# prs-eth/PCAccumulation

Hardware: AMD Instinct MI355X
Metric: LiDAR-frames/sec (5-frame seq, 160k pts) fwd+bwd (higher is better)
Workload: dtype mixed

## Files before the change

### include/pcacc.h

```cpp
#ifndef PCACC_H_
#define PCACC_H_

#include <stddef.h>
#include <stdint.h>

#ifdef __cplusplus
extern "C" {
#endif

#define PCACC_OK 0
#define PCACC_E_ARG (-1)
#define PCACC_E_WORKSPACE (-2)
#define PCACC_E_LAUNCH (-3)

#define PCACC_F32 0
#define PCACC_BF16 1

const char *pcacc_target(void);

int pcacc_cat2_rows(const void *a, int32_t a_row_bytes, const void *b, int32_t b_row_bytes, int64_t rows, void *out, void *stream);

int pcacc_reload_switches(void);

int pcacc_voxelize_workspace_bytes(int64_t n, int nx, int ny, int nz, int nt, size_t *bytes );
// ... 330 lines not shown

int pcacc_frames_max(const void *x, int dtype, int64_t n_seq, int32_t frames, int64_t plane, void *out, uint8_t *arg, void *stream);
int pcacc_frames_max_backward(const void *grad_out, const uint8_t *arg, int dtype, int64_t n_seq, int32_t frames, int64_t plane,
                              void *grad_x, void *stream);

int pcacc_bn_rows_workspace_bytes(int64_t rows, int32_t c, size_t *bytes );
int pcacc_bn_rows_forward(const void *x, int dtype, int64_t rows, int32_t c, const float *gamma, const float *beta, float eps,
                          float momentum, float *running_mean, float *running_var, void *y, float *save_mean,
                          float *save_invstd, void *workspace, size_t workspace_bytes, void *stream);
int pcacc_bn_rows_backward(const void *grad_y, const void *x, int dtype, int64_t rows, int32_t c, const float *gamma,
                           const float *save_mean, const float *save_invstd, void *grad_x, float *grad_gamma, float *grad_beta,
                           void *workspace, size_t workspace_bytes, void *stream);

int pcacc_bn_relu_rows_forward(const void *x, int dtype, int64_t rows, int32_t c, const float *gamma, const float *beta, float eps,
                               float momentum, float *running_mean, float *running_var, void *y, float *save_mean, float *save_invstd,
                               void *workspace, size_t workspace_bytes, void *stream);
int pcacc_bn_relu_rows_backward(const void *grad_y, const void *x, int dtype, int64_t rows, int32_t c, const float *gamma, const float *beta,
                                const float *save_mean, const float *save_invstd, void *grad_x, float *grad_gamma, float *grad_beta,
                                void *workspace, size_t workspace_bytes, void *stream);
int pcacc_bn_rows_forward_dual(const float *x, int64_t rows, int32_t c, const float *gamma, const float *beta, float eps, float momentum,
                               float *running_mean, float *running_var, int32_t relu, float *y, uint16_t *y16, float *y_amax, float *save_mean,
                               float *save_invstd, void *workspace, size_t workspace_bytes, void *stream);

int pcacc_bn_rows_backward_m(const void *grad_y, const void *x, int dtype, int64_t rows, int32_t c, const float *gamma, const float *beta,
                             int32_t relu, const float *save_mean, const float *save_invstd, void *grad_x, float *grad_x_amax, float *grad_gamma,
                             float *grad_beta, void *workspace, size_t workspace_bytes, void *stream);

int pcacc_pfn_block_forward(const uint16_t *xa, const uint16_t *pooled, const int32_t *p2v, const float *w0, const float *b0,
                            const float *ws, const float *w1, const float *b1, uint16_t *out, uint16_t *relu_h, int64_t rows, void *stream);
int pcacc_pfn_block_backward_workspace_bytes(int64_t rows, size_t *bytes );
int pcacc_pfn_block_backward(const uint16_t *xa, const uint16_t *pooled, const int32_t *p2v, const uint16_t *relu_h,
                             const uint16_t *grad_out, const float *w0, const float *ws, const float *w1, uint16_t *grad_xa,
                             uint16_t *grad_xb, float *grad_params, int64_t rows, void *workspace, size_t workspace_bytes, void *stream);

int pcacc_pfn_block_split_forward(const float *xa, const float *xa_amax, const float *pooled, const float *pooled_amax, const int32_t *p2v,
                                  const float *w0, const float *b0, const float *ws, const float *w1, const float *b1, float *out,
                                  float *relu_h, uint64_t *xmask, uint32_t *hmask, float *out_amax, float *hr_amax, int64_t rows,
                                  void *stream);
int pcacc_pfn_block_split_forward_dual(const float *xa, const float *xa_amax, const float *pooled, const float *pooled_amax, const int32_t *p2v,
                                       const float *w0, const float *b0, const float *ws, const float *w1, const float *b1, float *out,
                                       uint16_t *out16, uint16_t *hr16, float *out_amax, int64_t rows, void *stream);
int pcacc_pfn_block_split_dgrad(const float *grad_out, const float *grad_out_amax, const uint64_t *xmask, const uint32_t *hmask,
                                const float *w0, const float *ws, const float *w1, float *grad_xa, float *grad_xb, float *grad_h,
                                float *gx_amax, float *dh_amax, int64_t rows, void *stream);

int pcacc_maxpool2x2_bf16(const uint16_t *x, int64_t n_img, int32_t h, int32_t w, int32_t c, uint16_t *out, void *stream);
int pcacc_pool_skip_relu_backward_bf16(const uint16_t *y, const uint16_t *grad_pooled, const uint16_t *grad_skip, int64_t n_img, int32_t h,
                                       int32_t w, int32_t c, uint16_t *grad_y, void *stream);
int pcacc_maxpool2x2_f32(const float *x, int64_t n_img, int32_t h, int32_t w, int32_t c, float *out, void *stream);
int pcacc_pool_skip_relu_backward_f32(const float *y, const float *grad_pooled, const float *grad_skip, int64_t n_img, int32_t h, int32_t w,
                                      int32_t c, float *grad_y, float *out_amax, void *stream);
int pcacc_pool_skip_relu_backward_strided_bf16(const uint16_t *y, const uint16_t *grad_pooled, const uint16_t *grad_skip, int64_t skip_pitch,
                                               int64_t n_img, int32_t h, int32_t w, int32_t c, uint16_t *grad_y, void *stream);
int pcacc_pool_skip_relu_backward_strided_f32(const float *y, const float *grad_pooled, const float *grad_skip, int64_t skip_pitch,
                                              int64_t n_img, int32_t h, int32_t w, int32_t c, float *grad_y, float *out_amax, void *stream);
int pcacc_pool_skip_relu_backward_strided_y32(const float *y, const uint16_t *grad_pooled, const uint16_t *grad_skip, int64_t skip_pitch,
                                              int64_t n_img, int32_t h, int32_t w, int32_t c, uint16_t *grad_y, void *stream);

int pcacc_inv4x4(const float *m, int64_t n, float *out, void *stream);

int pcacc_rows_wgrad_few_supported(int32_t k, int32_t n);
int pcacc_rows_wgrad_few_workspace_bytes(int64_t rows, int32_t k, int32_t n, size_t *bytes );
int pcacc_rows_wgrad_few(const void *dy, const void *dy_mask, const void *x, int32_t x_relu, int64_t rows, int32_t k, int32_t n,
                         float *dw_aug, int32_t dtypes, void *workspace, size_t workspace_bytes, void *stream);

int pcacc_tube_rows(const float *xyz, const int32_t *slot, const float *slot_centre, int64_t n, int32_t n_frames, float *rows, void *stream);
int pcacc_tube_code(const float *geo, const float *motion, const float *frame, int64_t n_inst, int32_t n_frames, int32_t c, float *code,
                    void *stream);
int pcacc_tube_code_backward(const float *grad_code, int64_t n_inst, int32_t n_frames, int32_t c, float *grad_geo, float *grad_motion,
                             float *grad_frame, void *stream);
int pcacc_tube_pose_forward(const float *pose_vec, const float *remaining, const float *total_in, const float *slot_centre,
                            const float *weights, int32_t n_slots, int32_t n_frames, float *pose_c, float *gt_c, float *step,
                            float *remaining_out, float *total_out, double *loss_rt, float *wsum, void *stream);
int pcacc_tube_gap_forward(const float *rows, const int32_t *slot, const float *pose_c, const float *gt_c, int64_t n, float *pp, void *stream);
int pcacc_tube_finish(const float *slot_sums, int32_t stride, const float *count, const float *weights, const float *wsum, int32_t n_slots,
                      float *l12, void *stream);
int pcacc_tube_gap_backward(const float *rows, const int32_t *slot, const float *pose_c, const float *gt_c, const float *weights,
                            const float *count, const float *wsum, const float *grad_l1, const float *grad_l2, int64_t n,
                            float *grad_rows16, void *stream);
int pcacc_tube_pose_backward(const float *pose_vec, const float *remaining, const float *slot_centre, const float *weights, const float *wsum,
                             const float *grad_pose, int32_t stride, const double *grad_rot, const double *grad_trans, int32_t n_slots,
                             int32_t n_frames, float *grad_vec, void *stream);

int pcacc_upload_words(const uint32_t *host_words, int64_t n, uint32_t *dst, void *stream);

#ifdef __cplusplus
}
#endif
#endif
```

### pcaccumulation_amd/native.py

```python
import ctypes
import os
import re

import torch

_HERE = os.path.dirname(os.path.abspath(__file__))
LIB_PATH = os.environ.get('PCACC_LIB') or os.path.join(_HERE, 'csrc', 'libpcacc_hip.so')

F32, BF16 = 0, 1
_ERR = {-1: 'PCACC_E_ARG', -2: 'PCACC_E_WORKSPACE', -3: 'PCACC_E_LAUNCH'}

_lib = None


class NativeError(RuntimeError):
    pass


_CTYPES = {'int': ctypes.c_int, 'int32_t': ctypes.c_int, 'int64_t': ctypes.c_int64, 'uint64_t': ctypes.c_uint64, 'size_t': ctypes.c_size_t,
           'float': ctypes.c_float, 'double': ctypes.c_double}


def _prototypes():
    text = re.sub(r'/\*.*?\*/', '', open(os.path.join(_HERE, os.pardir, 'include', 'pcacc.h')).read(), flags=re.S)
# ... 1379 lines not shown
    _check(lib().pcacc_bn_rows_backward(_dev(grad_y, None, 'grad_y'), _dev(x, None, 'x'), _dtype_code(x), rows, int(c),
                                        _opt(gamma, torch.float32, 'gamma'), _dev(save_mean, torch.float32), _dev(save_invstd, torch.float32),
                                        _dev(gx), _dev(gg), _dev(gb), _dev(ws), ws.numel(), _stream()), 'bn_rows_backward')
    return gx, gg, gb


def tube_rows(xyz, slot, slot_centre, n_frames):
    n = xyz.shape[0]
    rows = torch.empty((n, 4), dtype=torch.float32, device=xyz.device)
    _check(lib().pcacc_tube_rows(_dev(xyz, torch.float32, 'xyz'), _dev(slot, torch.int32, 'slot'), _dev(slot_centre, torch.float32, 'slot_centre'),
                                 n, int(n_frames), _dev(rows), _stream()), 'tube_rows')
    return rows


def tube_code(geo, motion, frame, n_frames):
    n_inst, c = geo.shape
    code = torch.empty((n_inst * n_frames, 4 * c), dtype=torch.float32, device=geo.device)
    _check(lib().pcacc_tube_code(_dev(geo, torch.float32, 'geo'), _dev(motion, torch.float32, 'motion'), _dev(frame, torch.float32, 'frame'),
                                 n_inst, int(n_frames), int(c), _dev(code), _stream()), 'tube_code')
    return code


def tube_code_backward(grad_code, n_inst, n_frames, c):
    dev = grad_code.device
    g_geo = torch.empty((n_inst, c), dtype=torch.float32, device=dev)
    g_motion = torch.empty((n_inst, c), dtype=torch.float32, device=dev)
    g_frame = torch.empty((n_inst * n_frames, c), dtype=torch.float32, device=dev)
    _check(lib().pcacc_tube_code_backward(_dev(grad_code, torch.float32, 'grad_code'), n_inst, int(n_frames), int(c), _dev(g_geo),
                                          _dev(g_motion), _dev(g_frame), _stream()), 'tube_code_backward')
    return g_geo, g_motion, g_frame


def tube_pose_forward(pose_vec, remaining, total, slot_centre, weights, n_frames):
    s = pose_vec.shape[0]
    dev = pose_vec.device
    f = lambda *shape: torch.empty(shape, dtype=torch.float32, device=dev)
    pose_c, gt_c, step, rem_out, total_out, wsum = f(s, 12), f(s, 12), f(s, 4, 4), f(s, 4, 4), f(s, 4, 4), f(1)
    loss_rt = torch.empty((2,), dtype=torch.float64, device=dev)
    _check(lib().pcacc_tube_pose_forward(_dev(pose_vec, torch.float32, 'pose_vec'), _dev(remaining, torch.float32, 'remaining'),
                                         _opt(total, torch.float32, 'total'), _dev(slot_centre, torch.float32, 'slot_centre'),
                                         _dev(weights, torch.float32, 'weights'), int(s), int(n_frames), _dev(pose_c), _dev(gt_c), _dev(step),
                                         _dev(rem_out), _dev(total_out), _dev(loss_rt), _dev(wsum), _stream()), 'tube_pose_forward')
    return pose_c, gt_c, step, rem_out, total_out, loss_rt, wsum


def tube_gap_forward(rows, slot, pose_c, gt_c):
    n = rows.shape[0]
    pp = torch.empty((n, 4), dtype=torch.float32, device=rows.device)
    _check(lib().pcacc_tube_gap_forward(_dev(rows, torch.float32, 'rows'), _dev(slot, torch.int32, 'slot'), _dev(pose_c, torch.float32, 'pose_c'),
                                        _dev(gt_c, torch.float32, 'gt_c'), n, _dev(pp), _stream()), 'tube_gap_forward')
    return pp


def tube_finish(slot_sums, count, weights, wsum):
    l12 = torch.empty((2,), dtype=torch.float32, device=slot_sums.device)
    _check(lib().pcacc_tube_finish(_dev(slot_sums, torch.float32, 'slot_sums'), int(slot_sums.shape[1]), _dev(count, torch.float32, 'count'),
                                   _dev(weights, torch.float32, 'weights'), _dev(wsum, torch.float32, 'wsum'), int(slot_sums.shape[0]),
                                   _dev(l12), _stream()), 'tube_finish')
    return l12


def tube_gap_backward(rows, slot, pose_c, gt_c, weights, count, wsum, grad_l1, grad_l2):
    n = rows.shape[0]
    g16 = torch.empty((n, 16), dtype=torch.float32, device=rows.device)
    _check(lib().pcacc_tube_gap_backward(_dev(rows, torch.float32, 'rows'), _dev(slot, torch.int32, 'slot'), _dev(pose_c, torch.float32, 'pose_c'),
                                         _dev(gt_c, torch.float32, 'gt_c'), _dev(weights, torch.float32, 'weights'),
                                         _dev(count, torch.float32, 'count'), _dev(wsum, torch.float32, 'wsum'),
                                         _opt(grad_l1, torch.float32, 'grad_l1'), _opt(grad_l2, torch.float32, 'grad_l2'), n, _dev(g16),
                                         _stream()), 'tube_gap_backward')
    return g16


def tube_pose_backward(pose_vec, remaining, slot_centre, weights, wsum, grad_pose, grad_rot, grad_trans, n_frames):
    s = pose_vec.shape[0]
    g_vec = torch.empty((s, 7), dtype=torch.float32, device=pose_vec.device)
    _check(lib().pcacc_tube_pose_backward(_dev(pose_vec, torch.float32, 'pose_vec'), _dev(remaining, torch.float32, 'remaining'),
                                          _dev(slot_centre, torch.float32, 'slot_centre'), _dev(weights, torch.float32, 'weights'),
                                          _dev(wsum, torch.float32, 'wsum'), _dev(grad_pose, torch.float32, 'grad_pose'), int(grad_pose.shape[1]),
                                          _opt(grad_rot, torch.float64, 'grad_rot'), _opt(grad_trans, torch.float64, 'grad_trans'), int(s),
                                          int(n_frames), _dev(g_vec), _stream()), 'tube_pose_backward')
    return g_vec


def maxpool2x2(x_rows):
    n, h, w, c = x_rows.shape
    out = torch.empty((n, h // 2, w // 2, c), dtype=x_rows.dtype, device=x_rows.device)
    if x_rows.dtype == torch.float32:
        _check(lib().pcacc_maxpool2x2_f32(_dev(x_rows, torch.float32, 'x'), n, int(h), int(w), int(c), _dev(out), _stream()), 'maxpool2x2')
    else:
        _check(lib().pcacc_maxpool2x2_bf16(_dev(x_rows, torch.bfloat16, 'x'), n, int(h), int(w), int(c), _dev(out), _stream()), 'maxpool2x2')
    return out


def _pixel_pitch(g, shape):
    n, h, w, c = shape
    if tuple(g.shape) != tuple(shape) or g.stride(3) != 1:
        return None
    p = g.stride(2)
    if p < c or g.stride(1) != w * p or g.stride(0) != h * w * p or g.data_ptr() % 16:
        return None
    return p


def pool_skip_relu_backward(y_rows, grad_pooled, grad_skip, want_amax=False):
    n, h, w, c = y_rows.shape
    if y_rows.dtype == torch.float32 and any(g is not None and g.dtype == torch.bfloat16 for g in (grad_pooled, grad_skip)):
        out = torch.empty(y_rows.shape, dtype=torch.bfloat16, device=y_rows.device)
        pitch, gs_ptr = c, None
        if grad_skip is not None:
            pitch = _pixel_pitch(grad_skip, y_rows.shape)
            if pitch is None or pitch % 8:
                grad_skip, pitch = grad_skip.contiguous(), c
            gs_ptr = ctypes.c_void_p(grad_skip.data_ptr())
        _check(lib().pcacc_pool_skip_relu_backward_strided_y32(_dev(y_rows, torch.float32, 'y'), _opt(grad_pooled, torch.bfloat16, 'grad_pooled'), gs_ptr,
                                                               pitch, n, int(h), int(w), int(c), _dev(out), _stream()), 'pool_skip_relu_backward')
        return out
    out = torch.empty_like(y_rows)
    f32 = y_rows.dtype == torch.float32
    dt = torch.float32 if f32 else torch.bfloat16
    pitch, gs_ptr = c, None
    if grad_skip is not None:
        if grad_skip.dtype != dt or not grad_skip.is_cuda:
            raise NativeError('pool_skip_relu_backward: grad_skip must be a %s GPU tensor' % dt)
        pitch = _pixel_pitch(grad_skip, y_rows.shape)
        if pitch is None or pitch % (4 if f32 else 8):
            grad_skip, pitch = grad_skip.contiguous(), c
        gs_ptr = ctypes.c_void_p(grad_skip.data_ptr())
    if f32:
        amax = _zero256(y_rows.device) if want_amax else None
        _check(lib().pcacc_pool_skip_relu_backward_strided_f32(_dev(y_rows, torch.float32, 'y'), _opt(grad_pooled, torch.float32, 'grad_pooled'), gs_ptr,
                                                               pitch, n, int(h), int(w), int(c), _dev(out),
                                                               _dev(amax) if want_amax else None, _stream()), 'pool_skip_relu_backward')
        return (out, amax) if want_amax else out
    _check(lib().pcacc_pool_skip_relu_backward_strided_bf16(_dev(y_rows, torch.bfloat16, 'y'), _opt(grad_pooled, torch.bfloat16, 'grad_pooled'), gs_ptr,
                                                            pitch, n, int(h), int(w), int(c), _dev(out), _stream()), 'pool_skip_relu_backward')
    return out


PFN_BLOCK_SLICES = {'w1': (0, 1024, (32, 32)), 'b1': (1024, 1056, (32,)), 'ws': (1056, 3104, (32, 64)), 'w0': (3104, 5152, (32, 64)),
                    'b0': (5152, 5184, (32,))}


def pfn_block_forward(xa, pooled, p2v, w0, b0, ws, w1, b1):
    rows = xa.shape[0]
    out = torch.empty((rows, 32), dtype=torch.bfloat16, device=xa.device)
    hr = torch.empty((rows, 32), dtype=torch.bfloat16, device=xa.device)
    _check(lib().pcacc_pfn_block_forward(_dev(xa, torch.bfloat16, 'xa'), _opt(pooled, torch.bfloat16, 'pooled'), _opt(p2v, torch.int32, 'p2v'),
                                         _dev(w0, torch.float32, 'w0'), _opt(b0, torch.float32, 'b0'), _dev(ws, torch.float32, 'ws'),
                                         _dev(w1, torch.float32, 'w1'), _opt(b1, torch.float32, 'b1'), _dev(out), _dev(hr), rows, _stream()), 'pfn_block_forward')
    return out, hr


def pfn_block_backward(xa, pooled, p2v, hr, grad_out, w0, ws, w1):
    rows = xa.shape[0]
    dev = xa.device
    two = pooled is not None
    gxa = torch.empty((rows, 32 if two else 64), dtype=torch.bfloat16, device=dev)
    gxb = torch.empty((rows, 32), dtype=torch.bfloat16, device=dev) if two else None
    gp = torch.empty((5184,), dtype=torch.float32, device=dev)
    ws_buf = _workspace(lib().pcacc_pfn_block_backward_workspace_bytes, dev, rows)
    _check(lib().pcacc_pfn_block_backward(_dev(xa, torch.bfloat16, 'xa'), _opt(pooled, torch.bfloat16, 'pooled'), _opt(p2v, torch.int32, 'p2v'),
                                          _dev(hr, torch.bfloat16, 'relu_h'), _dev(grad_out, torch.bfloat16, 'grad_out'),
                                          _dev(w0, torch.float32, 'w0'), _dev(ws, torch.float32, 'ws'), _dev(w1, torch.float32, 'w1'),
                                          _dev(gxa), _opt(gxb, torch.bfloat16, 'grad_xb'), _dev(gp), rows, _dev(ws_buf),
                                          ws_buf.numel(), _stream()), 'pfn_block_backward')
    return gxa, gxb, gp
# ... 134 lines not shown
```

### pcaccumulation_amd/ops.py

```python
import weakref

import os

import torch

from . import native


class PillarIndex(object):

    def __init__(self, coordinates, point_to_voxel_map, batch_size, input_shape, cell_order=False):
        nx, ny, nz, nt = (int(v) for v in input_shape[:4])
        self.nx, self.ny, self.nt, self.batch_size = nx, ny, nt, int(batch_size)
        self.m = int(coordinates.shape[0])
        self.n_cells = self.batch_size * nt * ny * nx
        self.cells_per_frame = ny * nx
        coords = coordinates.contiguous()
        if coords.dtype not in (torch.float64, torch.int32):
            coords = coords.to(torch.float64)
        self.cell, self.cell2pillar = native.cell_index(coords, nx, ny, nt, self.batch_size)
        self.coordinates, self.perm, self._frames = coordinates, None, None
        p2v = point_to_voxel_map
        if p2v is not None:
            p2v = (p2v[:, 0] if p2v.dim() == 2 else p2v).to(torch.int32)
# ... 912 lines not shown
    def forward(ctx, points, idx, tsfm):
        tsfm = tsfm.detach().clone()
        ctx.save_for_backward(points, idx, tsfm)
        return native.rigid_transform(points, idx, tsfm.reshape(-1, 16))

    @staticmethod
    def backward(ctx, g):
        points, idx, tsfm = ctx.saved_tensors
        g = g.contiguous()
        gp = gt = None
        if ctx.needs_input_grad[0]:
            rt = torch.zeros_like(tsfm)
            rt[:, :3, :3] = tsfm[:, :3, :3].transpose(1, 2)
            gp = native.rigid_transform(g, idx, rt.reshape(-1, 16).contiguous())
        if ctx.needs_input_grad[2]:
            hom = torch.cat([points, torch.ones_like(points[:, :1])], dim=1)
            outer = (g[:, :, None] * hom[:, None, :]).reshape(-1, 12)
            rows = scatter(outer, idx, dim=0, dim_size=tsfm.shape[0], reduce='sum')
            gt = torch.zeros_like(tsfm)
            gt[:, :3, :] = rows.view(-1, 3, 4)
        return gp, None, gt


def transform_by_index(points, idx, tsfm):
    out = _TransformByIndex.apply(points.contiguous().float(), idx.to(torch.int32).contiguous(), tsfm.contiguous().float())
    return out if points.dtype == torch.float32 else out.to(points.dtype)


def _plan_sum(x, plan):
    if plan.small(x.shape[1]):
        return native.scatter_sum_small(x, plan.p2v, plan.m)
    return native.segment_sum(x, plan.seg_offsets, plan.order, plan.m)


def tube_rows(xyz, plan, slot_centre, n_frames):
    return native.tube_rows(xyz.detach().contiguous().float(), plan.p2v, slot_centre.detach().contiguous().float(), n_frames)


class _TubeCode(torch.autograd.Function):
    @staticmethod
    def forward(ctx, geo, motion, frame, n_frames):
        ctx.dims = (geo.shape[0], n_frames, geo.shape[1])
        return native.tube_code(geo.contiguous(), motion.contiguous(), frame.contiguous(), n_frames)

    @staticmethod
    def backward(ctx, grad):
        g_geo, g_motion, g_frame = native.tube_code_backward(grad.contiguous(), *ctx.dims)
        return g_geo, g_motion, g_frame, None


def tube_code(geo, motion, frame, n_frames):
    return _TubeCode.apply(geo.float(), motion.float(), frame.float(), int(n_frames))


class _TubePose(torch.autograd.Function):

    @staticmethod
    def forward(ctx, pose_vec, rows, plan, remaining, total, slot_centre, weights, n_frames):
        pose_vec = pose_vec.contiguous().float()
        remaining = remaining.detach().contiguous().float().view(-1, 4, 4)
        total = total.detach().contiguous().float().view(-1, 4, 4) if total is not None else None
        pose_c, gt_c, step, rem_out, total_out, loss_rt, wsum = native.tube_pose_forward(pose_vec, remaining, total, slot_centre, weights, n_frames)
        count = plan.count()
        l12 = native.tube_finish(_plan_sum(native.tube_gap_forward(rows, plan.p2v, pose_c, gt_c), plan), count, weights, wsum)
        ctx.save_for_backward(pose_vec, rows, remaining, slot_centre, weights, pose_c, gt_c, count, wsum)
        ctx.plan, ctx.n_frames = plan, n_frames
        ctx.mark_non_differentiable(step, rem_out, total_out)
        return l12[0], l12[1], loss_rt[0], loss_rt[1], step, rem_out, total_out

    @staticmethod
    def backward(ctx, g_l1, g_l2, g_rot, g_trans, *unused):
        pose_vec, rows, remaining, slot_centre, weights, pose_c, gt_c, count, wsum = ctx.saved_tensors
        plan = ctx.plan
        c = lambda g, dt: g.contiguous().to(dt) if g is not None else None
        g16 = native.tube_gap_backward(rows, plan.p2v, pose_c, gt_c, weights, count, wsum, c(g_l1, torch.float32), c(g_l2, torch.float32))
        g_vec = native.tube_pose_backward(pose_vec, remaining, slot_centre, weights, wsum, _plan_sum(g16, plan), c(g_rot, torch.float64),
                                          c(g_trans, torch.float64), ctx.n_frames)
        return g_vec, None, None, None, None, None, None, None


def tube_pose(pose_vec, rows, plan, remaining, total, slot_centre, weights, n_frames):
    return _TubePose.apply(pose_vec, rows, plan, remaining, total, slot_centre.detach().contiguous().float(), weights.detach().contiguous().float(),
                           int(n_frames))


_PREPARED = {}
_WEIGHT_EPOCH = 0


def weights_may_have_changed():
    global _WEIGHT_EPOCH
    _WEIGHT_EPOCH += 1


_ALL_OPTIMIZERS_WATCHED = False


def watch_all_optimizers():
    global _ALL_OPTIMIZERS_WATCHED
    if not _ALL_OPTIMIZERS_WATCHED:
        from torch.optim.optimizer import register_optimizer_step_post_hook
        register_optimizer_step_post_hook(lambda *a, **k: weights_may_have_changed())
        _ALL_OPTIMIZERS_WATCHED = True


def _weight_key(weight):
    return (weight._version, weight.data_ptr(), _WEIGHT_EPOCH)


def _weight_ref(cache, key, weight):
    return weakref.ref(weight, lambda _r, c=cache, k=key: c.pop(k, None))


_BATCH_ON = os.environ.get('PCACC_BATCH_PREPARE', '1') != '0'
_BATCH_SEEN = {}
_BATCH_STATE = {}


def _batch_note(weight, kind):
    k = (id(weight), kind)
    if _BATCH_ON and k not in _BATCH_SEEN and weight.is_cuda and weight.dtype == torch.float32:
        _BATCH_SEEN[k] = weakref.ref(weight, lambda _r, k=k: _BATCH_SEEN.pop(k, None))


def _batch_build(dev, live):
    import numpy as np
    jobs = np.zeros((len(live), 16), dtype=np.int64)
    forms, b0 = [], 0
    for row, (ref, w, kind) in zip(jobs, live):
        st = w.stride()
        if kind == 1:
            a, b, kt = w.shape[0], w.shape[1], 1
            fwd = (torch.empty((2, 4 * b, a), dtype=torch.float16, device=dev), torch.empty((4 * b,), dtype=torch.float32, device=dev))
            bwd = (torch.empty((2, a, 4 * b), dtype=torch.float16, device=dev), torch.empty((a,), dtype=torch.float32, device=dev))
            strides, blocks = (st[0], st[1], 0, st[2], st[3]), 4 * b + a
        elif kind == 3:
            a, b, kt = w.shape[0], w.shape[1], 1
            fwd = torch.empty((4 * b, a), dtype=torch.bfloat16, device=dev)
            bwd = torch.empty((a, 4 * b), dtype=torch.bfloat16, device=dev)
            strides, blocks = (st[0], st[1], 0, st[2], st[3]), min(512, max(1, (8 * a * b + 2047) // 2048))
        else:
            a, b, kt = w.shape[0], w.shape[1], (3 if w.dim() == 5 else 1)
            strides = tuple(st) if kt == 3 else (st[0], st[1], 0, st[2], st[3])
            if kind == 0:
                fwd = (torch.empty((2, kt * 9, a, b), dtype=torch.float16, device=dev), torch.empty((a,), dtype=torch.float32, device=dev))
                bwd = (torch.empty((2, kt * 9, b, a), dtype=torch.float16, device=dev), torch.empty((b,), dtype=torch.float32, device=dev))
                blocks = a + b
            else:
                fwd = torch.empty((kt * 9, a, b), dtype=torch.bfloat16, device=dev)
                bwd = torch.empty((kt * 9, b, a), dtype=torch.bfloat16, device=dev)
                blocks = min(512, max(1, (2 * kt * 9 * a * b + 2047) // 2048))
        ptrs = (fwd[0].data_ptr(), fwd[1].data_ptr(), bwd[0].data_ptr(), bwd[1].data_ptr()) if kind < 2 else (fwd.data_ptr(), 0, bwd.data_ptr(), 0)
        row[:] = (w.data_ptr(),) + ptrs + strides + (a, b, kt, kind, b0, blocks)
        b0 += blocks
        forms.append((ref, kind, fwd, bwd))
    return {'jobs': torch.from_numpy(jobs).to(dev), 'n': len(live), 'blocks': b0, 'forms': forms}


def _batch_refresh(dev):
    state = _BATCH_STATE.get(dev.index)
    if state is not None and state['epoch'] == _WEIGHT_EPOCH:
        return False
    live = []
    for (_, kind), ref in list(_BATCH_SEEN.items()):
        w = ref()
        if w is not None and w.is_cuda and w.device == dev and w.dtype == torch.float32:
# ... 899 lines not shown
```

### pcaccumulation_amd/tpointnet.py

```python
import torch
import torch.nn as nn
import torch.nn.functional as F

from .chamfer_distance import ChamferDistance
from . import ops
from .ops import scatter, ScatterPlan, linear_rows, transform_by_index, point_dtype, tube_rows, tube_code, tube_pose

_EPS = 1e-20


_CONST = {}


def _const(name, device, build):
    key = (name, str(device))
    if key not in _CONST:
        _CONST[key] = build().to(device)
    return _CONST[key]


def _quat_products_to_pose():
    x, y, z, w = 0, 1, 2, 3
    rot = {(0, 0): [(w, w, 1), (x, x, 1), (y, y, -1), (z, z, -1)], (0, 1): [(x, y, 2), (w, z, -2)], (0, 2): [(w, y, 2), (x, z, 2)],
           (1, 0): [(w, z, 2), (x, y, 2)], (1, 1): [(w, w, 1), (x, x, -1), (y, y, 1), (z, z, -1)], (1, 2): [(y, z, 2), (w, x, -2)],
# ... 124 lines not shown
    layers = []
    for i in range(len(dims) - 1):
        layers.append(nn.Linear(dims[i], dims[i + 1], bias=True))
        if i < len(dims) - 2:
            layers.append(nn.ReLU())
    return nn.Sequential(*layers)


def _embed(seq, x):
    mods = list(seq)
    i = 0
    pd = point_dtype() if x.is_cuda else x.dtype
    if pd != x.dtype and mods[0].in_features >= 32:
        x = x.to(pd)
    head = False
    n_lin = sum(isinstance(m, nn.Linear) for m in mods)
    if ops.mixed_mode() and x.is_cuda and x.dtype == torch.float32 and x.shape[0] >= ops.MIN_ROWS_FUSED_LINEAR and n_lin > 1:
        if mods[0].in_features >= 32:
            x = ops.enter_mixed(x.contiguous())
        else:
            head = True
    k = 0
    while i < len(mods):
        relu = i + 1 < len(mods) and isinstance(mods[i + 1], nn.ReLU)
        k += 1
        if k == n_lin:
            x = ops.exit_mixed(x)
        x = linear_rows(x, mods[i], post_relu=relu, out_dtype=pd, mixed=head and i == 0)
        i += 2 if relu else 1
    return x


class TPointNet(BaseModel):

    def __init__(self, config):
        BaseModel.__init__(self, config)
        self.geo_embed = _mlp([32, 32, 64, 128])
        self.motion_embed = _mlp([64, 64, 128, 128])
        self.pos_embed = _mlp([4, 32, 64, 128])
        self.regressor = nn.Sequential(nn.Linear(512, 256), nn.BatchNorm1d(256), nn.ReLU(),
                                       nn.Linear(256, 128), nn.BatchNorm1d(128), nn.ReLU(), nn.Linear(128, 7))
        self.min_points_per_frame = config['tpointnet']['min_points']

    def _frame_weights(self, slot, per_slot, moving, n_inst, n_slots, device):
        ones = torch.ones(slot.size(0), device=device)
        population = scatter(ones, slot, dim=0, dim_size=n_slots, reduce='sum', plan=per_slot)
        enough = (population > self.min_points_per_frame).float()
        slot_label = scatter(moving, slot, dim=0, dim_size=n_slots, reduce='max', plan=per_slot)
        label_w = torch.ones_like(slot_label)
        label_w[slot_label == 0] = 0.2
        ramp = (torch.arange(self.n_frames, device=device) + 1).repeat(n_inst) / self.n_frames
        return enough * label_w * ramp

    def shared_terms(self, input_dict):
        feats_motion, feats_geo = input_dict['mos_feats'], input_dict['frame_feats']
        t_idx, inst = input_dict['time_indice'], input_dict['inst_labels']
        n_inst, T = input_dict['inst_motion_gt'].size(0), input_dict['inst_motion_gt'].size(1)
        n_slots = n_inst * T
        slot = (inst * T + t_idx).long()
        per_slot = ScatterPlan(slot, n_slots)
        per_inst = ScatterPlan(inst, n_inst)
        weights = self._frame_weights(slot, per_slot, input_dict['mos_labels'], n_inst, n_slots, feats_motion.device)
        e_motion = scatter(_embed(self.motion_embed, feats_motion), inst, dim=0, dim_size=n_inst, reduce='max', plan=per_inst)
        e_geo = scatter(_embed(self.geo_embed, feats_geo), inst, dim=0, dim_size=n_inst, reduce='max', plan=per_inst)
        return {'slot': slot, 'per_slot': per_slot, 'per_inst': per_inst, 'weights': weights,
                'e_motion': e_motion.float(), 'e_geo': e_geo.float()}

    def _frame_embedding(self, xyz, slot, per_slot, n_slots, T):
        slot_centre = scatter(xyz, slot, dim=0, dim_size=n_slots, reduce='mean', plan=per_slot)
        rows = tube_rows(xyz, per_slot, slot_centre, T)
        e_frame = scatter(_embed(self.pos_embed, rows), slot, dim=0, dim_size=n_slots, reduce='max', plan=per_slot)
        return e_frame.float(), slot_centre, rows

    def forward(self, input_dict, shared=None):
        xyz = input_dict['points']
        gt_motion = input_dict['inst_motion_gt']
        n_inst, T = gt_motion.size(0), gt_motion.size(1)
        n_slots = n_inst * T
        if shared is None:
            shared = self.shared_terms(input_dict)
        slot, per_slot, weights = shared['slot'], shared['per_slot'], shared['weights']
        e_frame, slot_centre, rows = self._frame_embedding(xyz, slot, per_slot, n_slots, T)

        pose_vec = self.regressor(tube_code(shared['e_geo'], shared['e_motion'], e_frame, T))

        l1_loss, l2_loss, rot_loss, trans_loss, step, remaining, total = tube_pose(
            pose_vec, rows, per_slot, gt_motion, input_dict.get('total'), slot_centre, weights, T)
        shape = (n_inst, T, 4, 4)
        return {'l1_loss': l1_loss, 'l2_loss': l2_loss, 'rot_loss': rot_loss, 'trans_loss': trans_loss,
                'inst_est_motion': step.view(shape), 'remaining': remaining.view(shape), 'total': total.view(shape)}
```

Baseline: 668.0.

## Fuse tube regressor MLP with BatchNorm and ReLU into custom HIP kernels

```diff
diff --git a/include/pcacc.h b/include/pcacc.h
--- a/include/pcacc.h
+++ b/include/pcacc.h
@@ -436,6 +436,18 @@
                              const float *grad_pose, int32_t stride, const double *grad_rot, const double *grad_trans, int32_t n_slots,
                              int32_t n_frames, float *grad_vec, void *stream);
 
+int pcacc_tube_regressor_forward(const float *x, int64_t m, const float *w1, const float *b1, const float *gamma1, const float *beta1, float eps1,
+                                 float momentum1, float *running_mean1, float *running_var1, int64_t *num_batches_tracked1, const float *w2,
+                                 const float *b2, const float *gamma2, const float *beta2, float eps2, float momentum2, float *running_mean2,
+                                 float *running_var2, int64_t *num_batches_tracked2, const float *w3, const float *b3, float *z1, float *y1,
+                                 float *mean1, float *invstd1, float *z2, float *y2, float *mean2, float *invstd2, float *pose, void *stream);
+int pcacc_tube_regressor_backward(const float *grad_pose, const float *x, int64_t m, const float *w1, const float *gamma1, const float *w2,
+                                  const float *gamma2, const float *w3, const float *z1, const float *y1, const float *mean1,
+                                  const float *invstd1, const float *z2, const float *y2, const float *mean2, const float *invstd2, float *gz1,
+                                  float *gz2, float *grad_x, float *grad_w1, float *grad_b1, float *grad_gamma1, float *grad_beta1,
+                                  float *grad_w2, float *grad_b2, float *grad_gamma2, float *grad_beta2, float *grad_w3, float *grad_b3,
+                                  void *stream);
+
 int pcacc_upload_words(const uint32_t *host_words, int64_t n, uint32_t *dst, void *stream);
 
 #ifdef __cplusplus
diff --git a/pcaccumulation_amd/csrc/tube_regressor.hip b/pcaccumulation_amd/csrc/tube_regressor.hip
--- /dev/null
+++ b/pcaccumulation_amd/csrc/tube_regressor.hip
@@ -0,0 +1,322 @@
+#include "common.h"
+
+#define TR_THREADS 256
+#define TR_NJ 4
+#define TR_MAX_ROWS ((int64_t)1 << 24)
+
+template <int N>
+__device__ __forceinline__ void tr_block_sum(double (&v)[N], double *red)
+{
+#pragma unroll
+    for (int n = 0; n < N; ++n) {
+        double s = v[n];
+#pragma unroll
+        for (int d = 32; d; d >>= 1) s += __shfl_xor(s, d, 64);
+        if ((threadIdx.x & 63) == 0) red[(threadIdx.x >> 6) * N + n] = s;
+    }
+    __syncthreads();
+#pragma unroll
+    for (int n = 0; n < N; ++n) v[n] = (red[n] + red[N + n]) + (red[2 * N + n] + red[3 * N + n]);
+    __syncthreads();
+}
+
+__device__ __forceinline__ float tr_sum4(const float (&a)[4]) { return (a[0] + a[1]) + (a[2] + a[3]); }
+
+template <int K>
+__device__ __forceinline__ void tr_dot_rows(const float *__restrict__ row, const float *__restrict__ w, float (&out)[TR_NJ])
+{
+    float acc[TR_NJ][4];
+#pragma unroll
+    for (int j = 0; j < TR_NJ; ++j) acc[j][0] = acc[j][1] = acc[j][2] = acc[j][3] = 0.f;
+    const float4 *r4 = reinterpret_cast<const float4 *>(row);
+#pragma unroll 4
+    for (int k4 = 0; k4 < K / 4; ++k4) {
+        const float4 xv = r4[k4];
+#pragma unroll
+        for (int j = 0; j < TR_NJ; ++j) {
+            const float4 wv = reinterpret_cast<const float4 *>(w + j * K)[k4];
+            acc[j][0] = fmaf(xv.x, wv.x, acc[j][0]);
+            acc[j][1] = fmaf(xv.y, wv.y, acc[j][1]);
+            acc[j][2] = fmaf(xv.z, wv.z, acc[j][2]);
+            acc[j][3] = fmaf(xv.w, wv.w, acc[j][3]);
+        }
+    }
+#pragma unroll
+    for (int j = 0; j < TR_NJ; ++j) out[j] = tr_sum4(acc[j]);
+}
+
+template <int CN>
+__device__ __forceinline__ void tr_dot_cols(const float *__restrict__ row, const float *__restrict__ w, int ldw, float (&out)[TR_NJ])
+{
+    if (CN % 4 == 0) {
+        float acc[4][TR_NJ];
+#pragma unroll
+        for (int p = 0; p < 4; ++p) acc[p][0] = acc[p][1] = acc[p][2] = acc[p][3] = 0.f;
+        const float4 *r4 = reinterpret_cast<const float4 *>(row);
+#pragma unroll 2
+        for (int c4 = 0; c4 < CN / 4; ++c4) {
+            const float4 gv = r4[c4];
+            const float g[4] = {gv.x, gv.y, gv.z, gv.w};
+#pragma unroll
+            for (int p = 0; p < 4; ++p) {
+                const float4 wv = *reinterpret_cast<const float4 *>(w + (int64_t)(c4 * 4 + p) * ldw);
+                acc[p][0] = fmaf(g[p], wv.x, acc[p][0]);
+                acc[p][1] = fmaf(g[p], wv.y, acc[p][1]);
+                acc[p][2] = fmaf(g[p], wv.z, acc[p][2]);
+                acc[p][3] = fmaf(g[p], wv.w, acc[p][3]);
+            }
+        }
+#pragma unroll
+        for (int j = 0; j < TR_NJ; ++j) out[j] = (acc[0][j] + acc[1][j]) + (acc[2][j] + acc[3][j]);
+    } else {
+#pragma unroll
+        for (int j = 0; j < TR_NJ; ++j) out[j] = 0.f;
+#pragma unroll
+        for (int c = 0; c < CN; ++c) {
+            const float g = row[c];
+            const float4 wv = *reinterpret_cast<const float4 *>(w + (int64_t)c * ldw);
+            out[0] = fmaf(g, wv.x, out[0]);
+            out[1] = fmaf(g, wv.y, out[1]);
+            out[2] = fmaf(g, wv.z, out[2]);
+            out[3] = fmaf(g, wv.w, out[3]);
+        }
+    }
+}
+
+__device__ __forceinline__ float4 tr_ld4(const float *p, int64_t i) { return *reinterpret_cast<const float4 *>(p + i); }
+__device__ __forceinline__ void tr_st4(float *p, int64_t i, const float (&v)[4]) { *reinterpret_cast<float4 *>(p + i) = make_float4(v[0], v[1], v[2], v[3]); }
+
+template <int K>
+__global__ __launch_bounds__(TR_THREADS) void tr_layer_fwd_kernel(const float *__restrict__ x, int64_t m, int c, const float *__restrict__ w,
+                                                                  const float *__restrict__ b, const float *__restrict__ gamma,
+                                                                  const float *__restrict__ beta, float eps, float momentum, float *running_mean,
+                                                                  float *running_var, int64_t *num_batches_tracked, float *z, float *__restrict__ y,
+                                                                  float *__restrict__ mean_out, float *__restrict__ invstd_out)
+{
+    __shared__ double red[4 * TR_NJ];
+    const int j0 = blockIdx.x * TR_NJ;
+    const float *w0 = w + (int64_t)j0 * K;
+    double s[TR_NJ] = {0., 0., 0., 0.};
+    for (int64_t r = threadIdx.x; r < m; r += TR_THREADS) {
+        float zv[TR_NJ];
+        tr_dot_rows<K>(x + r * K, w0, zv);
+#pragma unroll
+        for (int j = 0; j < TR_NJ; ++j) {
+            zv[j] += b[j0 + j];
+            s[j] += zv[j];
+        }
+        tr_st4(z, r * c + j0, zv);
+    }
+    tr_block_sum<TR_NJ>(s, red);
+    const double n = (double)m;
+    float mean[TR_NJ];
+    double q[TR_NJ] = {0., 0., 0., 0.};
+#pragma unroll
+    for (int j = 0; j < TR_NJ; ++j) mean[j] = (float)(s[j] / n);
+    for (int64_t r = threadIdx.x; r < m; r += TR_THREADS) {
+        const float4 t = tr_ld4(z, r * c + j0);
+        const float zv[4] = {t.x, t.y, t.z, t.w};
+#pragma unroll
+        for (int j = 0; j < TR_NJ; ++j) q[j] += (double)(zv[j] - mean[j]) * (double)(zv[j] - mean[j]);
+    }
+    tr_block_sum<TR_NJ>(q, red);
+    float invstd[TR_NJ], ga[TR_NJ], be[TR_NJ];
+#pragma unroll
+    for (int j = 0; j < TR_NJ; ++j) {
+        q[j] /= n;
+        invstd[j] = 1.f / sqrtf((float)q[j] + eps);
+        ga[j] = gamma[j0 + j];
+        be[j] = beta[j0 + j];
+    }
+    for (int64_t r = threadIdx.x; r < m; r += TR_THREADS) {
+        const float4 t = tr_ld4(z, r * c + j0);
+        const float zv[4] = {t.x, t.y, t.z, t.w};
+        float yv[TR_NJ];
+#pragma unroll
+        for (int j = 0; j < TR_NJ; ++j) {
+            const float v = (zv[j] - mean[j]) * invstd[j] * ga[j] + be[j];
+            yv[j] = v > 0.f ? v : (v == v ? 0.f : v);
+        }
+        tr_st4(y, r * c + j0, yv);
+    }
+#pragma unroll
+    for (int j = 0; j < TR_NJ; ++j)
+        if (threadIdx.x == j) {
+            mean_out[j0 + j] = mean[j];
+            invstd_out[j0 + j] = invstd[j];
+            if (running_mean) running_mean[j0 + j] = (1.f - momentum) * running_mean[j0 + j] + momentum * mean[j];
+            if (running_var) running_var[j0 + j] = (1.f - momentum) * running_var[j0 + j] + momentum * (float)(q[j] * (n / (n - 1.)));
+        }
+    if (num_batches_tracked && blockIdx.x == 0 && threadIdx.x == 0) *num_batches_tracked += 1;
+}
+
+__global__ __launch_bounds__(64) void tr_pose_kernel(const float *__restrict__ y2, int64_t m, const float *__restrict__ w3, const float *__restrict__ b3,
+                                                     float *__restrict__ pose)
+{
+    const int64_t i = (int64_t)blockIdx.x * 64 + threadIdx.x;
+    if (i >= m * 7) return;
+    const int64_t r = i / 7;
+    const int p = (int)(i - r * 7);
+    float acc[4] = {0.f, 0.f, 0.f, 0.f};
+#pragma unroll 8
+    for (int k4 = 0; k4 < 32; ++k4) {
+        const float4 a = tr_ld4(y2, r * 128 + k4 * 4), wv = tr_ld4(w3, p * 128 + k4 * 4);
+        acc[0] = fmaf(a.x, wv.x, acc[0]);
+        acc[1] = fmaf(a.y, wv.y, acc[1]);
+        acc[2] = fmaf(a.z, wv.z, acc[2]);
+        acc[3] = fmaf(a.w, wv.w, acc[3]);
+    }
+    pose[i] = tr_sum4(acc) + b3[p];
+}
+
+template <int CN, int K>
+__global__ __launch_bounds__(TR_THREADS) void tr_layer_bwd_kernel(const float *__restrict__ gnext, const float *__restrict__ wnext,
+                                                                  const float *__restrict__ z, const float *__restrict__ y,
+                                                                  const float *__restrict__ xin, const float *__restrict__ mean,
+                                                                  const float *__restrict__ invstd, const float *__restrict__ gamma, int64_t m, int c,
+                                                                  float *gz, float *__restrict__ dw, float *__restrict__ db,
+                                                                  float *__restrict__ dgamma, float *__restrict__ dbeta, float *__restrict__ dw_last,
+                                                                  float *__restrict__ db_last)
+{
+    __shared__ double red[4 * 2 * TR_NJ];
+    if ((int)blockIdx.x >= c / TR_NJ) {
+        const int p = blockIdx.x - c / TR_NJ;
+        double s[1] = {0.};
+        for (int64_t r = threadIdx.x; r < m; r += TR_THREADS) s[0] += gnext[r * CN + p];
+        tr_block_sum<1>(s, red);
+        if (threadIdx.x == 0) db_last[p] = (float)s[0];
+        for (int k = threadIdx.x; k < c; k += TR_THREADS) {
+            float acc[4] = {0.f, 0.f, 0.f, 0.f};
+            int64_t r = 0;
+            for (; r + 3 < m; r += 4) {
+#pragma unroll
+                for (int u = 0; u < 4; ++u) acc[u] = fmaf(gnext[(r + u) * CN + p], y[(r + u) * c + k], acc[u]);
+            }
+            for (; r < m; ++r) acc[0] = fmaf(gnext[r * CN + p], y[r * c + k], acc[0]);
+            dw_last[p * c + k] = tr_sum4(acc);
+        }
+        return;
+    }
+    const int j0 = blockIdx.x * TR_NJ;
+    const double n = (double)m;
+    float mu[TR_NJ], is[TR_NJ];
+#pragma unroll
+    for (int j = 0; j < TR_NJ; ++j) mu[j] = mean[j0 + j], is[j] = invstd[j0 + j];
+    double s[2 * TR_NJ] = {0., 0., 0., 0., 0., 0., 0., 0.};
+    for (int64_t r = threadIdx.x; r < m; r += TR_THREADS) {
+        float gn[TR_NJ];
+        tr_dot_cols<CN>(gnext + r * CN, wnext + j0, c, gn);
+        const float4 yt = tr_ld4(y, r * c + j0), zt = tr_ld4(z, r * c + j0);
+        const float yv[4] = {yt.x, yt.y, yt.z, yt.w}, zv[4] = {zt.x, zt.y, zt.z, zt.w};
+#pragma unroll
+        for (int j = 0; j < TR_NJ; ++j) {
+            gn[j] = yv[j] > 0.f ? gn[j] : 0.f;
+            s[j] += gn[j];
+            s[TR_NJ + j] += (double)gn[j] * (double)((zv[j] - mu[j]) * is[j]);
+        }
+        tr_st4(gz, r * c + j0, gn);
+    }
+    tr_block_sum<2 * TR_NJ>(s, red);
+    float sc[TR_NJ], mb[TR_NJ], mg[TR_NJ];
+    double t[TR_NJ] = {0., 0., 0., 0.};
+#pragma unroll
+    for (int j = 0; j < TR_NJ; ++j) sc[j] = gamma[j0 + j] * is[j], mb[j] = (float)(s[j] / n), mg[j] = (float)(s[TR_NJ + j] / n);
+    for (int64_t r = threadIdx.x; r < m; r += TR_THREADS) {
+        const float4 gt = tr_ld4(gz, r * c + j0), zt = tr_ld4(z, r * c + j0);
+        const float gn[4] = {gt.x, gt.y, gt.z, gt.w}, zv[4] = {zt.x, zt.y, zt.z, zt.w};
+        float g[TR_NJ];
+#pragma unroll
+        for (int j = 0; j < TR_NJ; ++j) {
+            g[j] = sc[j] * (gn[j] - mb[j] - (zv[j] - mu[j]) * is[j] * mg[j]);
+            t[j] += g[j];
+        }
+        tr_st4(gz, r * c + j0, g);
+    }
+    tr_block_sum<TR_NJ>(t, red);
+#pragma unroll
+    for (int j = 0; j < TR_NJ; ++j)
+        if (threadIdx.x == j) {
+            dbeta[j0 + j] = (float)s[j];
+            dgamma[j0 + j] = (float)s[TR_NJ + j];
+            db[j0 + j] = (float)t[j];
+        }
+    for (int k = threadIdx.x; k < K; k += TR_THREADS) {
+        float acc[4][TR_NJ];
+#pragma unroll
+        for (int u = 0; u < 4; ++u) acc[u][0] = acc[u][1] = acc[u][2] = acc[u][3] = 0.f;
+        int64_t r = 0;
+        for (; r + 3 < m; r += 4) {
+#pragma unroll
+            for (int u = 0; u < 4; ++u) {
+                const float4 g = tr_ld4(gz, (r + u) * c + j0);
+                const float xv = xin[(r + u) * K + k];
+                acc[u][0] = fmaf(g.x, xv, acc[u][0]);
+                acc[u][1] = fmaf(g.y, xv, acc[u][1]);
+                acc[u][2] = fmaf(g.z, xv, acc[u][2]);
+                acc[u][3] = fmaf(g.w, xv, acc[u][3]);
+            }
+        }
+        for (; r < m; ++r) {
+            const float4 g = tr_ld4(gz, r * c + j0);
+            const float xv = xin[r * K + k];
+            acc[0][0] = fmaf(g.x, xv, acc[0][0]);
+            acc[0][1] = fmaf(g.y, xv, acc[0][1]);
+            acc[0][2] = fmaf(g.z, xv, acc[0][2]);
+            acc[0][3] = fmaf(g.w, xv, acc[0][3]);
+        }
+#pragma unroll
+        for (int j = 0; j < TR_NJ; ++j) dw[(int64_t)(j0 + j) * K + k] = (acc[0][j] + acc[1][j]) + (acc[2][j] + acc[3][j]);
+    }
+}
+
+template <int C, int K>
+__global__ __launch_bounds__(TR_THREADS) void tr_gx_kernel(const float *__restrict__ gz, const float *__restrict__ w, int64_t m, float *__restrict__ gx)
+{
+    const int j0 = blockIdx.x * TR_NJ;
+    for (int64_t r = threadIdx.x; r < m; r += TR_THREADS) {
+        float g[TR_NJ];
+        tr_dot_cols<C>(gz + r * C, w + j0, K, g);
+        tr_st4(gx, r * K + j0, g);
+    }
+}
+
+extern "C" int pcacc_tube_regressor_forward(const float *x, int64_t m, const float *w1, const float *b1, const float *gamma1, const float *beta1, float eps1,
+                                            float momentum1, float *running_mean1, float *running_var1, int64_t *num_batches_tracked1, const float *w2,
+                                            const float *b2, const float *gamma2, const float *beta2, float eps2, float momentum2, float *running_mean2,
+                                            float *running_var2, int64_t *num_batches_tracked2, const float *w3, const float *b3, float *z1, float *y1,
+                                            float *mean1, float *invstd1, float *z2, float *y2, float *mean2, float *invstd2, float *pose, void *stream)
+{
+    if (!x || !w1 || !b1 || !gamma1 || !beta1 || !w2 || !b2 || !gamma2 || !beta2 || !w3 || !b3 || !z1 || !y1 || !mean1 || !invstd1 || !z2 || !y2 || !mean2 ||
+        !invstd2 || !pose)
+        return PCACC_E_ARG;
+    if (m < 2 || m > TR_MAX_ROWS) return PCACC_E_ARG;
+    hipStream_t s = pcacc_stream(stream);
+    tr_layer_fwd_kernel<512><<<256 / TR_NJ, TR_THREADS, 0, s>>>(x, m, 256, w1, b1, gamma1, beta1, eps1, momentum1, running_mean1, running_var1,
+                                                                num_batches_tracked1, z1, y1, mean1, invstd1);
+    tr_layer_fwd_kernel<256><<<128 / TR_NJ, TR_THREADS, 0, s>>>(y1, m, 128, w2, b2, gamma2, beta2, eps2, momentum2, running_mean2, running_var2,
+                                                                num_batches_tracked2, z2, y2, mean2, invstd2);
+    tr_pose_kernel<<<(int)((m * 7 + 63) / 64), 64, 0, s>>>(y2, m, w3, b3, pose);
+    PCACC_CHECK_LAUNCH();
+    return PCACC_OK;
+}
+
+extern "C" int pcacc_tube_regressor_backward(const float *grad_pose, const float *x, int64_t m, const float *w1, const float *gamma1, const float *w2,
+                                             const float *gamma2, const float *w3, const float *z1, const float *y1, const float *mean1,
+                                             const float *invstd1, const float *z2, const float *y2, const float *mean2, const float *invstd2, float *gz1,
+                                             float *gz2, float *grad_x, float *grad_w1, float *grad_b1, float *grad_gamma1, float *grad_beta1,
+                                             float *grad_w2, float *grad_b2, float *grad_gamma2, float *grad_beta2, float *grad_w3, float *grad_b3,
+                                             void *stream)
+{
+    if (!grad_pose || !x || !w1 || !gamma1 || !w2 || !gamma2 || !w3 || !z1 || !y1 || !mean1 || !invstd1 || !z2 || !y2 || !mean2 || !invstd2 || !gz1 || !gz2 ||
+        !grad_w1 || !grad_b1 || !grad_gamma1 || !grad_beta1 || !grad_w2 || !grad_b2 || !grad_gamma2 || !grad_beta2 || !grad_w3 || !grad_b3)
+        return PCACC_E_ARG;
+    if (m < 2 || m > TR_MAX_ROWS) return PCACC_E_ARG;
+    hipStream_t s = pcacc_stream(stream);
+    tr_layer_bwd_kernel<7, 256><<<128 / TR_NJ + 7, TR_THREADS, 0, s>>>(grad_pose, w3, z2, y2, y1, mean2, invstd2, gamma2, m, 128, gz2, grad_w2, grad_b2,
+                                                                       grad_gamma2, grad_beta2, grad_w3, grad_b3);
+    tr_layer_bwd_kernel<128, 512><<<256 / TR_NJ, TR_THREADS, 0, s>>>(gz2, w2, z1, y1, x, mean1, invstd1, gamma1, m, 256, gz1, grad_w1, grad_b1, grad_gamma1,
+                                                                     grad_beta1, nullptr, nullptr);
+    if (grad_x) tr_gx_kernel<256, 512><<<512 / TR_NJ, TR_THREADS, 0, s>>>(gz1, w1, m, grad_x);
+    PCACC_CHECK_LAUNCH();
+    return PCACC_OK;
+}
diff --git a/pcaccumulation_amd/native.py b/pcaccumulation_amd/native.py
--- a/pcaccumulation_amd/native.py
+++ b/pcaccumulation_amd/native.py
@@ -1485,6 +1485,40 @@
     return g_vec
 
 
+def tube_regressor_forward(x, w1, b1, bn1, w2, b2, bn2, w3, b3):
+    m, dev = x.shape[0], x.device
+    f = lambda *shape: torch.empty(shape, dtype=torch.float32, device=dev)
+    z1, y1, mean1, invstd1, z2, y2, mean2, invstd2, pose = f(m, 256), f(m, 256), f(256), f(256), f(m, 128), f(m, 128), f(128), f(128), f(m, 7)
+    g1, be1, eps1, mom1, rm1, rv1, nbt1 = bn1
+    g2, be2, eps2, mom2, rm2, rv2, nbt2 = bn2
+    _check(lib().pcacc_tube_regressor_forward(_dev(x, torch.float32, 'x'), m, _dev(w1, torch.float32, 'w1'), _dev(b1, torch.float32, 'b1'),
+                                              _dev(g1, torch.float32, 'gamma1'), _dev(be1, torch.float32, 'beta1'), eps1, mom1,
+                                              _opt(rm1, torch.float32, 'running_mean1'), _opt(rv1, torch.float32, 'running_var1'),
+                                              _opt(nbt1, torch.int64, 'num_batches_tracked1'), _dev(w2, torch.float32, 'w2'),
+                                              _dev(b2, torch.float32, 'b2'), _dev(g2, torch.float32, 'gamma2'), _dev(be2, torch.float32, 'beta2'), eps2,
+                                              mom2, _opt(rm2, torch.float32, 'running_mean2'), _opt(rv2, torch.float32, 'running_var2'),
+                                              _opt(nbt2, torch.int64, 'num_batches_tracked2'), _dev(w3, torch.float32, 'w3'),
+                                              _dev(b3, torch.float32, 'b3'), _dev(z1), _dev(y1), _dev(mean1), _dev(invstd1), _dev(z2), _dev(y2),
+                                              _dev(mean2), _dev(invstd2), _dev(pose), _stream()), 'tube_regressor_forward')
+    return pose, (z1, y1, mean1, invstd1, z2, y2, mean2, invstd2)
+
+
+def tube_regressor_backward(grad_pose, x, w1, g1, w2, g2, w3, saved, want_grad_x=True):
+    z1, y1, mean1, invstd1, z2, y2, mean2, invstd2 = saved
+    m, dev = x.shape[0], x.device
+    f = lambda *shape: torch.empty(shape, dtype=torch.float32, device=dev)
+    gz1, gz2, gx = f(m, 256), f(m, 128), (f(m, 512) if want_grad_x else None)
+    gw1, gb1, gg1, gbe1, gw2, gb2, gg2, gbe2, gw3, gb3 = f(256, 512), f(256), f(256), f(256), f(128, 256), f(128), f(128), f(128), f(7, 128), f(7)
+    _check(lib().pcacc_tube_regressor_backward(_dev(grad_pose, torch.float32, 'grad_pose'), _dev(x, torch.float32, 'x'), m, _dev(w1, torch.float32, 'w1'),
+                                               _dev(g1, torch.float32, 'gamma1'), _dev(w2, torch.float32, 'w2'), _dev(g2, torch.float32, 'gamma2'),
+                                               _dev(w3, torch.float32, 'w3'), _dev(z1, torch.float32), _dev(y1, torch.float32),
+                                               _dev(mean1, torch.float32), _dev(invstd1, torch.float32), _dev(z2, torch.float32),
+                                               _dev(y2, torch.float32), _dev(mean2, torch.float32), _dev(invstd2, torch.float32), _dev(gz1), _dev(gz2),
+                                               _opt(gx, torch.float32, 'grad_x'), _dev(gw1), _dev(gb1), _dev(gg1), _dev(gbe1), _dev(gw2), _dev(gb2),
+                                               _dev(gg2), _dev(gbe2), _dev(gw3), _dev(gb3), _stream()), 'tube_regressor_backward')
+    return gx, gw1, gb1, gg1, gbe1, gw2, gb2, gg2, gbe2, gw3, gb3
+
+
 def maxpool2x2(x_rows):
     n, h, w, c = x_rows.shape
     out = torch.empty((n, h // 2, w // 2, c), dtype=x_rows.dtype, device=x_rows.device)
diff --git a/pcaccumulation_amd/ops.py b/pcaccumulation_amd/ops.py
--- a/pcaccumulation_amd/ops.py
+++ b/pcaccumulation_amd/ops.py
@@ -1018,6 +1018,56 @@
 def tube_pose(pose_vec, rows, plan, remaining, total, slot_centre, weights, n_frames):
     return _TubePose.apply(pose_vec, rows, plan, remaining, total, slot_centre.detach().contiguous().float(), weights.detach().contiguous().float(),
                            int(n_frames))
+
+
+_TUBE_REGRESSOR = os.environ.get('PCACC_TUBE_REGRESSOR', '1') != '0'
+
+
+class _TubeRegressor(torch.autograd.Function):
+
+    @staticmethod
+    def forward(ctx, x, w1, b1, g1, be1, w2, b2, g2, be2, w3, b3, bn1, bn2):
+        x = x.contiguous()
+        tensors = [t.detach().contiguous() for t in (w1, b1, g1, be1, w2, b2, g2, be2, w3, b3)]
+        w1, b1, g1, be1, w2, b2, g2, be2, w3, b3 = tensors
+        stats = lambda bn: (bn.eps, bn.momentum, bn.running_mean, bn.running_var, bn.num_batches_tracked)
+        pose, saved = native.tube_regressor_forward(x, w1, b1, (g1, be1) + stats(bn1), w2, b2, (g2, be2) + stats(bn2), w3, b3)
+        ctx.save_for_backward(x, w1, g1, w2, g2, w3, *saved)
+        return pose
+
+    @staticmethod
+    def backward(ctx, grad_pose):
+        x, w1, g1, w2, g2, w3 = ctx.saved_tensors[:6]
+        grads = native.tube_regressor_backward(grad_pose.contiguous().float(), x, w1, g1, w2, g2, w3, ctx.saved_tensors[6:],
+                                               want_grad_x=ctx.needs_input_grad[0])
+        return grads + (None, None)
+
+
+def _tube_regressor_native(x, seq):
+    if not _TUBE_REGRESSOR or not seq.training or len(seq) != 7 or x.dim() != 2 or x.shape[0] < 2 or torch.is_autocast_enabled():
+        return False
+    kinds = (torch.nn.Linear, torch.nn.BatchNorm1d, torch.nn.ReLU, torch.nn.Linear, torch.nn.BatchNorm1d, torch.nn.ReLU, torch.nn.Linear)
+    if any(type(mod) is not kind for mod, kind in zip(seq, kinds)):
+        return False
+    if [(seq[i].in_features, seq[i].out_features) for i in (0, 3, 6)] != [(512, 256), (256, 128), (128, 7)] or x.shape[1] != 512:
+        return False
+    for lin in (seq[0], seq[3], seq[6]):
+        if lin.bias is None:
+            return False
+    for bn in (seq[1], seq[4]):
+        if not bn.training or not bn.affine or bn.momentum is None or not bn.track_running_stats or bn.running_mean is None:
+            return False
+    tensors = [x] + list(seq.parameters()) + [b for bn in (seq[1], seq[4]) for b in (bn.running_mean, bn.running_var)]
+    return all(t.is_cuda and t.dtype == torch.float32 and t.device == x.device for t in tensors) and all(
+        seq[i].num_batches_tracked.is_cuda and seq[i].num_batches_tracked.dtype == torch.int64 for i in (1, 4))
+
+
+def tube_regressor(x, seq):
+    if not _tube_regressor_native(x, seq):
+        return seq(x)
+    lin1, bn1, _, lin2, bn2, _, lin3 = seq
+    return _TubeRegressor.apply(x, lin1.weight, lin1.bias, bn1.weight, bn1.bias, lin2.weight, lin2.bias, bn2.weight, bn2.bias, lin3.weight, lin3.bias,
+                                bn1, bn2)
 
 
 _PREPARED = {}
diff --git a/pcaccumulation_amd/tpointnet.py b/pcaccumulation_amd/tpointnet.py
--- a/pcaccumulation_amd/tpointnet.py
+++ b/pcaccumulation_amd/tpointnet.py
@@ -230,7 +230,7 @@
         slot, per_slot, weights = shared['slot'], shared['per_slot'], shared['weights']
         e_frame, slot_centre, rows = self._frame_embedding(xyz, slot, per_slot, n_slots, T)
 
-        pose_vec = self.regressor(tube_code(shared['e_geo'], shared['e_motion'], e_frame, T))
+        pose_vec = ops.tube_regressor(tube_code(shared['e_geo'], shared['e_motion'], e_frame, T), self.regressor)
 
         l1_loss, l2_loss, rot_loss, trans_loss, step, remaining, total = tube_pose(
             pose_vec, rows, per_slot, gt_motion, input_dict.get('total'), slot_centre, weights, T)
```

Measured after the change: 660.8. -1.1%, worse.
